# bghira/universal-metal-flash-attention

Hardware: NVIDIA B200
Metric: attention forward TFLOP/s (higher is better)
Workload: dtype bf16

## Files before the change

### universal-metal-flash-attention_b200/csrc/attn_fwd_tc.cu

```cuda
#include <cuda.h>
#include <cuda_runtime.h>
#include <cuda_fp16.h>
#include <math_constants.h>

#include <mutex>
#include <type_traits>

#include "common.h"
#include "fwd_tc.h"
#include "sm100_ptx.cuh"
#include "tc_host.h"

namespace mfa {

namespace {

using namespace ptx;

constexpr int kThreads = 384;
constexpr float kLog2e = 1.4426950408889634f;
constexpr float kLn2 = 0.6931471805599453f;
constexpr float kRescaleThreshold = 8.f;
constexpr int kTileNoMask = 1 << 30;
constexpr int kParts = 4;

template <int D, int MODE, int MASKED = 0>
struct Cfg {
  static constexpr bool kI4 = MODE == kFwdI4 || MODE == kFwdI4F8;
  static constexpr bool kF8 = MODE == kFwdI8F8 || MODE == kFwdI4F8;
  static constexpr bool kI8 = MODE == kFwdI8 || kF8 || kI4;
  static constexpr bool kSplit = MODE == kFwdSplit;
  static constexpr bool kWide = MODE == kFwdWideF16 || MODE == kFwdWideBF16;
  static constexpr int kChunkBytes = 128 * 128;
  static constexpr int kQChunks = kI8 ? 1 : D / 64;
  static constexpr int kVChunks = kF8 ? 1 : D / 64;
  static constexpr int kHalf = kQChunks * kChunkBytes;
  static constexpr int kQTile = kHalf * ((kSplit || kWide) ? 2 : 1);
  static constexpr int kVTile = kVChunks * kChunkBytes;
  static constexpr int kStage = kVTile;
  static constexpr int kSPS = kSplit ? 4 : kWide ? 3 : 2;
  static constexpr bool kMaskTma = MASKED == 2 && (MODE == kFwdF16 || MODE == kFwdBF16);
  static constexpr int kMaskTile = 128 * 128 * 2;
  static constexpr bool kShallow = MASKED != 0 && !kI4;
  static constexpr int kStages = (kSplit || kWide) ? 3
                               : (D == 128 && !kF8) ? (kShallow ? 3 : 5) : (kShallow ? 6 : 10);
  static constexpr int kBarBytes = 112 + 16 * kStages + 16 + 16 + 64 + 32;
  static constexpr int kPoly = kSplit ? 0 : 3;
  static constexpr int kRawTile = 128 * 64, kRawStages = 3;
  static constexpr int kRawBytes = kI4 ? (kRawStages + 1) * kRawTile + 1024 + 128 : 0;
  static constexpr int kMaskBytes = kMaskTma ? 2 * kMaskTile + 1024 : 0;
  static constexpr int kSmem = 2 * kQTile + kStages * kStage + kBarBytes + kRawBytes + kMaskBytes + 1024;
  static_assert(kSmem <= 232448, "shared memory budget of one CTA");
};

__device__ __forceinline__ f32x2 exp2_poly2(f32x2 x) {
  float x0, x1;
  unpack2(x, x0, x1);
  x = pack2(fmaxf(x0, -127.f), fmaxf(x1, -127.f));
  const f32x2 magic = pack2(12582912.f, 12582912.f);
  const f32x2 xr = add2_rm(x, magic);
  const f32x2 f = sub2(x, sub2(xr, magic));
  f32x2 pz = fma2(f, pack2(0.07706582f, 0.07706582f), pack2(0.22764632f, 0.22764632f));
  pz = fma2(pz, f, pack2(0.69511649f, 0.69511649f));
  pz = fma2(pz, f, pack2(1.0f, 1.0f));
  float p0, p1, r0, r1;
  unpack2(pz, p0, p1);
  unpack2(xr, r0, r1);
  return pack2(__int_as_float(__float_as_int(p0) + (__float_as_int(r0) << 23)),
               __int_as_float(__float_as_int(p1) + (__float_as_int(r1) << 23)));
}

template <int PF, int NP>
__device__ __forceinline__ void exp_part(const float* s, f32x2 a2, f32x2 nk2, uint32_t* pk, f32x2& acc_a, f32x2& acc_b) {
  static_assert(NP == 0 || NP == 3, "exp2 mixes: all MUFU, or pairs 1, 4, 6 of every 8 on the polynomial");
  constexpr int kSel = NP == 3 ? 0x52 : 0x00;
  uint32_t half16[PF == 2 ? 16 : 1];
#pragma unroll
  for (int i = 0; i < 16; ++i) {
    const f32x2 x = fma2(pack2(s[2 * i], s[2 * i + 1]), a2, nk2);
    f32x2 pp;
    float p0, p1;
    if ((kSel >> (i & 7)) & 1) {
      pp = exp2_poly2(x);
    } else {
      float x0, x1;
      unpack2(x, x0, x1);
      pp = pack2(ex2(x0), ex2(x1));
    }
    if (i & 1) acc_b = add2(acc_b, pp); else acc_a = add2(acc_a, pp);
    unpack2(pp, p0, p1);
    if constexpr (PF == 2) half16[i] = pack_e4m3(p0, p1);
    else if constexpr (PF == 3) {
      const uint32_t h = pack_f16(p0, p1);
      const float2 hf = __half22float2(*reinterpret_cast<const __half2*>(&h));
      pk[i] = h;
      pk[16 + i] = pack_f16(p0 - hf.x, p1 - hf.y);
    }
    else pk[i] = PF == 1 ? pack_bf16(p0, p1) : pack_f16(p0, p1);
  }
  if constexpr (PF == 2) {
#pragma unroll
    for (int i = 0; i < 8; ++i) pk[i] = half16[2 * i] | (half16[2 * i + 1] << 16);
  }
}

template <int PF, int NP>
__device__ __forceinline__ void exp_phase(const float* s, float a0, float a1, float nk0, float nk1, uint32_t tS,
                                          uint32_t bar0, int lane, float& sum_lo, float& sum_hi) {
  constexpr int kW = PF == 2 ? 8 : 16;
  f32x2 acc[2][2] = {{pack2(0.f, 0.f), pack2(0.f, 0.f)}, {pack2(0.f, 0.f), pack2(0.f, 0.f)}};
  uint32_t pk[kParts][PF == 3 ? 32 : kW];
#pragma unroll
  for (int part = 0; part < kParts; ++part) {
    const bool hi = part >= kParts / 2;
    const float ah = hi ? a1 : a0, nk = hi ? nk1 : nk0;
    exp_part<PF, NP>(s + 32 * part, pack2(ah, ah), pack2(nk, nk), pk[part], acc[hi ? 1 : 0][0], acc[hi ? 1 : 0][1]);
    if (part > 0) {
      tmem_wait_st();
      tc_fence_before();
      __syncwarp();
      if (lane == 0) mbar_arrive(bar0 + 8 * (part - 1));
    }
    if constexpr (PF == 2) tmem_st_x8(tS + kW * part, pk[part]);
    else tmem_st_x16(tS + kW * part, pk[part]);
    if constexpr (PF == 3) tmem_st_x16(tS + 64 + kW * part, pk[part] + 16);
  }
  tmem_wait_st();
  tc_fence_before();
  __syncwarp();
  if (lane == 0) mbar_arrive(bar0 + 8 * (kParts - 1));
  float x0, x1;
  unpack2(add2(acc[0][0], acc[0][1]), x0, x1); sum_lo = x0 + x1;
  unpack2(add2(acc[1][0], acc[1][1]), x0, x1); sum_hi = x0 + x1;
}

template <bool BF>
__device__ __forceinline__ void add_mask_pair(float& s0, float& s1, uint32_t w, f32x2 cn2) {
  float lo, hi;
  if constexpr (BF) {
    lo = __uint_as_float(w << 16);
    hi = __uint_as_float(w & 0xffff0000u);
  } else {
    const float2 f = __half22float2(*reinterpret_cast<const __half2*>(&w));
    lo = f.x; hi = f.y;
  }
  unpack2(fma2(pack2(s0, s1), cn2, pack2(lo, hi)), s0, s1);
}

template <int D, int MODE, int MASKED>
__global__ void __launch_bounds__(kThreads, 1) fwd_tc_kernel(const __grid_constant__ FwdTcParams p) {
  using C = Cfg<D, MODE, MASKED>;
  constexpr bool I8 = C::kI8, F8 = C::kF8, SPLIT = C::kSplit, I4 = C::kI4, WIDE = C::kWide, MT = C::kMaskTma;
  constexpr int PF = SPLIT ? 3 : F8 ? 2 : ((MODE == kFwdF16 || MODE == kFwdWideF16) ? 0 : 1);
  constexpr float kShift = F8 ? 6.f : 0.f;
  constexpr float kThr = F8 ? 2.f : kRescaleThreshold;
  constexpr int QT = C::kQTile, HT = C::kHalf, VT = C::kVTile, STG = C::kStage, NS = C::kStages, CHB = C::kChunkBytes;
  constexpr int SPS = C::kSPS;
  constexpr int kWg2Regs = 40;
  extern __shared__ uint8_t smem_raw[];
  const uint32_t raw = smem_u32(smem_raw);
  const uint32_t base = (raw + 1023u) & ~1023u;
  const uint32_t sQ = base, sKV = base + 2 * QT, sBar = sKV + NS * STG;
  auto q_full = [&](int t) { return sBar + 8 * t; };
  auto s_full = [&](int t) { return sBar + 16 + 8 * t; };
  auto o_full = [&](int t) { return sBar + 32 + 8 * t; };
  auto p_part = [&](int t, int k) { return sBar + 48 + 8 * (t * kParts + k); };
  auto kv_full = [&](int s) { return sBar + 112 + 8 * s; };
  auto kv_empty = [&](int s) { return sBar + 112 + 8 * NS + 8 * s; };
  const uint32_t tmem_slot = sBar + 112 + 16 * NS;
  auto o_empty = [&](int t) { return sBar + 112 + 16 * NS + 16 + 8 * t; };
  constexpr int NR = C::kRawStages, RAW = C::kRawTile;
  auto raw_full = [&](int s) { return sBar + 112 + 16 * NS + 32 + 8 * s; };
  auto raw_empty = [&](int s) { return sBar + 112 + 16 * NS + 56 + 8 * s; };
  const uint32_t qraw_full = sBar + 112 + 16 * NS + 80, qraw_empty = sBar + 112 + 16 * NS + 88;
  const uint32_t sRawK = (sBar + C::kBarBytes + 127u) & ~127u, sRawQ = sRawK + NR * RAW, sQsum = sRawQ + RAW;
  auto mk_full = [&](int t) { return sBar + 112 + 16 * NS + 96 + 8 * t; };
  auto mk_empty = [&](int t) { return sBar + 112 + 16 * NS + 112 + 8 * t; };
  const uint32_t sMask = (sBar + C::kBarBytes + 1023u) & ~1023u;

  const int warp = __shfl_sync(0xffffffffu, threadIdx.x >> 5, 0), lane = threadIdx.x & 31;
  const int* const seg_q = MASKED ? nullptr : p.cu_q;
  const int* const seg_k = MASKED ? nullptr : p.cu_k;
  struct Item { int r0, h, b, hk, nt, j_lo, n, lid, half; };
  auto decode = [&](int w) {
    const int nqb = (p.Sq + 255) / 256;
    Item it;
    it.half = 0;
    if constexpr (WIDE) { it.half = w & 1; w >>= 1; }
    const int x = w % nqb, hb = w / nqb;
    const int qblk = p.causal ? nqb - 1 - x : x;
    it.h = hb % p.H; it.b = hb / p.H;
    it.hk = it.h / (p.H / p.Hkv);
    it.r0 = qblk * 256;
    it.nt = (it.r0 + 128 < p.Sq) ? 2 : 1;
    int klo, khi;
    block_key_range(p.causal, p.window, p.Sq, p.Skv, seg_q, seg_k, p.nseq, it.r0, min(it.r0 + 256, p.Sq), klo, khi);
    it.j_lo = klo >> 7;
    it.n = khi > klo ? ((khi + 127) >> 7) - it.j_lo : 0;
    it.lid = 0;
    if constexpr (MASKED) {
      if (p.mtiles) {
        it.lid = ((p.mask_sb ? it.b : 0) * (p.mask_sh ? p.H : 1) + (p.mask_sh ? it.h : 0)) * nqb + qblk;
        it.n = __ldg(p.mcounts + it.lid);
      }
    }
    return it;
  };
  auto tile_of = [&](const Item& im, int it) {
    if constexpr (MASKED) { if (p.mtiles) return __ldg(p.mtiles + (size_t)im.lid * p.m_nkt + it); }
    return im.j_lo + it;
  };

  if (threadIdx.x == 256) {
    for (int t = 0; t < 2; ++t) {
      mbar_init(q_full(t), 1); mbar_init(s_full(t), 1); mbar_init(o_full(t), 1);
      for (int k = 0; k < kParts; ++k) mbar_init(p_part(t, k), 4);
    }
    for (int s = 0; s < NS; ++s) { mbar_init(kv_full(s), 1); mbar_init(kv_empty(s), 2); }
    for (int t = 0; t < 2; ++t) mbar_init(o_empty(t), 4);
    if constexpr (I4) {
      for (int r = 0; r < NR; ++r) { mbar_init(raw_full(r), 1); mbar_init(raw_empty(r), 1); }
      mbar_init(qraw_full, 1); mbar_init(qraw_empty, 1);
    }
    if constexpr (MT) {
      for (int t = 0; t < 2; ++t) { mbar_init(mk_full(t), 1); mbar_init(mk_empty(t), 4); }
    }
    fence_mbar_init();
  }
  if (warp == 9) {
    if (lane == 0) { prefetch_tmap(&p.tq); prefetch_tmap(&p.tk); prefetch_tmap(&p.tv); }
    __syncwarp();
    tmem_alloc(tmem_slot, 512);
    tmem_relinquish();
  }
  tc_fence_before();
  __syncthreads();
  tc_fence_after();
  const uint32_t tmem = __shfl_sync(0xffffffffu, *reinterpret_cast<volatile uint32_t*>(smem_raw + (tmem_slot - raw)), 0);

  if (warp == 9) {
    reg_dealloc<kWg2Regs>();
    if (lane == 0) {
      const Item im = decode(blockIdx.x);
      const int r0 = im.r0, h = im.h, b = im.b, hk = im.hk, nt = im.nt, n = im.n;
      int kvi = 0;
      int kr = 0, nqraw = 0;
      auto load_half = [&](uint32_t dst, const CUtensorMap* m, uint32_t bar, int row, int head, int col0 = 0) {
#pragma unroll
        for (int c = 0; c < C::kQChunks; ++c) tma_load_4d(dst + c * CHB, m, bar, col0 + c * (I8 ? 128 : 64), row, head, b);
      };
      auto load_q = [&](int t2) {
        if constexpr (I4) {
          if (nqraw > 0) mbar_wait(qraw_empty, (nqraw - 1) & 1);
          mbar_arrive_expect_tx(qraw_full, RAW);
          tma_load_4d(sRawQ, &p.tq, qraw_full, 0, r0 + t2 * 128, h, b);
          ++nqraw;
          return;
        }
        mbar_arrive_expect_tx(q_full(t2), QT);
        load_half(sQ + t2 * QT, &p.tq, q_full(t2), r0 + t2 * 128, h);
        if constexpr (SPLIT) load_half(sQ + t2 * QT + HT, &p.tq2, q_full(t2), r0 + t2 * 128, h);
        if constexpr (WIDE) load_half(sQ + t2 * QT + HT, &p.tq, q_full(t2), r0 + t2 * 128, h, 128);
      };
      auto load_k = [&](const CUtensorMap* m, int row, int col0 = 0) {
        if constexpr (I4) {
          const int rs = kr % NR;
          mbar_wait(raw_empty(rs), ((kr / NR) & 1) ^ 1);
          mbar_arrive_expect_tx(raw_full(rs), RAW);
          tma_load_4d(sRawK + rs * RAW, m, raw_full(rs), 0, row, hk, b);
          ++kr; ++kvi;
          return;
        }
        const int s = kvi % NS;
        mbar_wait(kv_empty(s), ((kvi / NS) & 1) ^ 1);
        mbar_arrive_expect_tx(kv_full(s), HT);
        load_half(sKV + s * STG, m, kv_full(s), row, hk, col0);
        ++kvi;
      };
      auto load_v = [&](const CUtensorMap* m, int row, int col0 = 0) {
        const int s = kvi % NS;
        mbar_wait(kv_empty(s), ((kvi / NS) & 1) ^ 1);
        mbar_arrive_expect_tx(kv_full(s), VT);
#pragma unroll
        for (int c = 0; c < C::kVChunks; ++c) tma_load_4d(sKV + s * STG + c * CHB, m, kv_full(s), col0 + c * 64, row, hk, b);
        ++kvi;
      };
      if (n > 0) load_q(0);
      for (int it = 0; it < n; ++it) {
        const int row = (tile_of(im, it) & (kTileNoMask - 1)) * 128;
        if constexpr (SPLIT) load_k(&p.tk2, row);
        load_k(&p.tk, row);
        if constexpr (WIDE) load_k(&p.tk, row, 128);
        if (it == 0 && nt == 2) load_q(1);
        load_v(&p.tv, row, WIDE ? 128 * im.half : 0);
        if constexpr (SPLIT) load_v(&p.tv2, row);
      }
    }
  } else if (warp == 8 || warp == 10) {
    reg_dealloc<kWg2Regs>();
    const int t = (warp - 8) >> 1;
    constexpr uint32_t FMT = (PF == 0 || PF == 3) ? 0u : 1u;
    constexpr uint32_t IDESC_S = I4 ? make_idesc(2, 1, 0, 0, 0, 128, 128)
                               : I8 ? make_idesc(2, 1, 1, 0, 0, 128, 128)
                                    : make_idesc(1, FMT, FMT, 0, 0, 128, 128);
    constexpr uint32_t IDESC_O = F8 ? make_idesc(1, 0, 0, 0, 1, 128, D)
                                    : make_idesc(1, FMT, FMT, 0, 1, 128, D);
    const uint32_t q_lo = desc_lo(sQ, 16) + t * (QT >> 4), k_lo = desc_lo(sKV, 16), v_lo = desc_lo(sKV, CHB);
    const uint32_t tS = tmem + t * 128, tO = tmem + 256 + t * D;
    auto wait_full = [&](int idx) { mbar_wait(kv_full(idx % NS), (idx / NS) & 1); };
    auto issue_qk = [&](uint32_t a0, int idx, bool acc0) {
      const uint32_t b0 = k_lo + (idx % NS) * (STG >> 4);
#pragma unroll
      for (int kk = 0; kk < D / 16; ++kk) {
        const uint32_t off = ((kk >> 2) * CHB + (kk & 3) * 32) >> 4;
        mma_f16_ss_u(tS, a0 + off, kDescHiSw128, b0 + off, kDescHiSw128, IDESC_S, acc0 || kk > 0);
      }
    };
    auto issue_s = [&](int idx) {
      const uint32_t b0 = k_lo + (idx % NS) * (STG >> 4);
      if constexpr (I8) {
#pragma unroll
        for (int kk = 0; kk < 4; ++kk)
          mma_i8_ss_u(tS, q_lo + kk * 2, kDescHiSw128, b0 + kk * 2, kDescHiSw128, IDESC_S, kk > 0);
      } else {
        issue_qk(q_lo, idx, false);
      }
    };
    auto issue_o_part = [&](int idx, int part, bool acc) {
      const uint32_t b0 = v_lo + (idx % NS) * (STG >> 4);
      if constexpr (F8) {
        mma_f8_ts_u(tO, tS + part * 8, b0 + part * (4096 >> 4), kDescHiSw128, IDESC_O, (acc || part > 0) ? 1u : 0u);
      } else {
#pragma unroll
        for (int kk = 2 * part; kk < 2 * part + 2; ++kk) {
          mma_f16_ts_u(tO, tS + kk * 8, b0 + kk * (2048 >> 4), kDescHiSw128, IDESC_O, (acc || kk > 0) ? 1u : 0u);
          if constexpr (SPLIT) mma_f16_ts_u(tO, tS + 64 + kk * 8, b0 + kk * (2048 >> 4), kDescHiSw128, IDESC_O, 1u);
        }
      }
    };
    int pc = 0;
    int oe = 0;
    const int F = SPLIT ? p.flush_steps : 0;
    const Item im = decode(blockIdx.x);
    const int nt = im.nt, n = im.n;
    if (n > 0 && t < nt) {
      auto release = [&](int idx) { tc_commit_u(kv_empty(idx % NS)); if (nt == 1) tc_commit_u(kv_empty(idx % NS)); };
      auto do_s = [&](int idx) {
        wait_full(idx);
        tc_fence_after();
        if constexpr (SPLIT) {
          issue_qk(q_lo, idx, false);
          release(idx);
          wait_full(idx + 1);
          tc_fence_after();
          issue_qk(q_lo, idx + 1, true);
          issue_qk(q_lo + (HT >> 4), idx + 1, true);
          tc_commit_u(s_full(t));
          release(idx + 1);
        } else if constexpr (WIDE) {
          issue_qk(q_lo, idx, false);
          release(idx);
          wait_full(idx + 1);
          tc_fence_after();
          issue_qk(q_lo + (HT >> 4), idx + 1, true);
          tc_commit_u(s_full(t));
          release(idx + 1);
        } else {
          issue_s(idx);
          tc_commit_u(s_full(t));
          release(idx);
        }
      };
      mbar_wait(q_full(t), 0);
      do_s(0);
      for (int it = 0; it < n; ++it) {
        const int vi = SPS * it + (SPS == 2 ? 1 : 2), ki = SPS * (it + 1);
        wait_full(vi);
#pragma unroll
        for (int part = 0; part < kParts; ++part) {
          mbar_wait(p_part(t, part), pc & 1);
          const bool fresh = F > 0 ? (it % F == 0) : (it == 0);
          if (part == 0 && fresh && it > 0) { mbar_wait(o_empty(t), oe & 1); ++oe; }
          tc_fence_after();
          issue_o_part(vi, part, !fresh);
        }
        release(vi);
        if constexpr (SPLIT) {
          wait_full(vi + 1);
          tc_fence_after();
          const uint32_t b0 = v_lo + ((vi + 1) % NS) * (STG >> 4);
#pragma unroll
          for (int kk = 0; kk < 8; ++kk) mma_f16_ts_u(tO, tS + kk * 8, b0 + kk * (2048 >> 4), kDescHiSw128, IDESC_O, 1u);
          release(vi + 1);
        }
        if (it + 1 < n) do_s(ki);
        else tc_commit_u(o_full(t));
        ++pc;
      }
    }
  } else if (warp < 8) {
    reg_alloc<232>();
    const int t = warp >> 2;
    const int row = (warp & 3) * 32 + lane;
    const uint32_t lane_base = (uint32_t)((warp & 3) * 32) << 16;
    const uint32_t tS = tmem + lane_base + t * 128;
    const uint32_t tO = tmem + lane_base + 256 + t * D;
    int pc = 0;
    int mkc = 0;
    if (t == 1) named_bar_arrive(2, 256);
    const Item im = decode(blockIdx.x);
    const int r0 = im.r0, h = im.h, b = im.b, hk = im.hk, nt = im.nt, n = im.n;
    const int r = r0 + t * 128 + row;
    float m = -CUDART_INF_F, l = 0.f;
    int clo, chi;
    row_key_range(p.causal, p.window, p.Sq, p.Skv, seg_q, seg_k, p.nseq, r, clo, chi);
    --chi;
    float qsc = p.c;
    const float* ksp = nullptr;
    const float* vsp = nullptr;
    if constexpr (I8) {
      const int rq = min(r, p.Sq - 1);
      qsc = (p.qs ? p.qs[((size_t)b * p.H + h) * p.sq_ + rq / p.qbr] : p.qs1) * p.c;
      ksp = p.ks ? p.ks + ((size_t)b * p.Hkv + hk) * p.sk_ : nullptr;
      vsp = p.vs ? p.vs + ((size_t)b * p.Hkv + hk) * p.sv_ : nullptr;
    }
    if constexpr (SPLIT) qsc = p.c * __ldg(p.qs) * __ldg(p.ks);
    float sb_row = p.s_bias;
    float m_flush = -CUDART_INF_F;
    int nflush = 0;
    const int dv_row = p.dv > 0 ? p.dv : D;
    const bool v_blocks = I8 && !F8 && vsp != nullptr;
    const bool pingpong = nt == 2;

    if (t < nt) {
      float ksn0 = p.ks1, ksn1 = p.ks1, vsn0 = 1.f, vsn1 = 1.f;
      int jt_next = n > 0 ? tile_of(im, 0) : 0;
      auto fetch_scales = [&](int jt) {
        if constexpr (I8) {
          const int c0 = (jt & (kTileNoMask - 1)) * 128;
          if (ksp) {
            ksn0 = __ldg(ksp + min(c0 / p.kbr, p.nbk - 1));
            ksn1 = __ldg(ksp + min((c0 + 64) / p.kbr, p.nbk - 1));
// ... 26 lines not shown
        if constexpr (SPLIT) {
          if (p.flush_steps > 0 && it > 0 && it % p.flush_steps == 0) {
            const float fs = (nflush > 0 && m_flush != -CUDART_INF_F) ? ex2(m_flush - m) : 0.f;
            float4* fbuf = reinterpret_cast<float4*>(p.flush_buf) + ((size_t)blockIdx.x * 2 + t) * (size_t)(D / 4) * 128 + row;
#pragma unroll
            for (int ch = 0; ch < D / 32; ++ch) {
              uint32_t ou[32];
              tmem_ld_x32(tO + ch * 32, ou);
              tmem_wait_ld();
#pragma unroll
              for (int i = 0; i < 8; ++i) {
                float4* dst = fbuf + (size_t)(ch * 8 + i) * 128;
                float4 o4 = make_float4(0.f, 0.f, 0.f, 0.f);
                if (nflush > 0) o4 = *dst;
                *dst = make_float4(fmaf(o4.x, fs, __uint_as_float(ou[4 * i])), fmaf(o4.y, fs, __uint_as_float(ou[4 * i + 1])),
                                   fmaf(o4.z, fs, __uint_as_float(ou[4 * i + 2])), fmaf(o4.w, fs, __uint_as_float(ou[4 * i + 3])));
              }
            }
            tc_fence_before();
            __syncwarp();
            if (lane == 0) mbar_arrive(o_empty(t));
            m_flush = m;
            ++nflush;
          }
        }
        if constexpr (I4) {
          if (it == 0) {
            sb_row = p.s_bias + 8.f * (float)(int)ld_shared_u32(sQsum + t * 512 + row * 4);
            cb0 = -sb_row * a0;
            cb1 = -sb_row * a1;
          }
        }
        uint32_t su[128];
        tmem_ld_x32(tS, su);
        tmem_ld_x32(tS + 32, su + 32);
        tmem_ld_x32(tS + 64, su + 64);
        tmem_ld_x32(tS + 96, su + 96);
        tmem_wait_ld();
        float* s = reinterpret_cast<float*>(su);
        if (it + 1 < n) { jt_next = tile_of(im, it + 1); fetch_scales(jt_next); }
        if constexpr (I8) {
          const int smul = p.s_mul;
          const uint32_t sadd = p.s_add;
#pragma unroll
          for (int i = 0; i < 128; ++i) su[i] = su[i] * smul + sadd;
        }
        if (MT && !mask_noop) {
          if constexpr (MT) {
            mbar_wait(mk_full(t), mkc & 1);
            ++mkc;
            const uint32_t mrow = sMask + (uint32_t)t * C::kMaskTile + (uint32_t)row * 128u;
            const uint32_t sw = (uint32_t)(row & 7);
            if (p.mask_kind == kMaskBool) {
#pragma unroll
              for (int j = 0; j < 8; ++j) {
                float f0, f1, f2, f3;
                ld_shared_v4(mrow + (((uint32_t)j ^ sw) << 4), f0, f1, f2, f3);
                const uint32_t w4[4] = {__float_as_uint(f0), __float_as_uint(f1), __float_as_uint(f2), __float_as_uint(f3)};
#pragma unroll
                for (int k = 0; k < 16; ++k)
                  if (((w4[k >> 2] >> (8 * (k & 3))) & 0xffu) == 0) s[16 * j + k] = -CUDART_INF_F;
              }
            } else {
              const float cn = a0 * kLn2;
              const f32x2 cn2 = pack2(cn, cn);
              auto apply = [&](auto is_bf) {
#pragma unroll
                for (int g = 0; g < 2; ++g) {
#pragma unroll
                  for (int j = 0; j < 8; ++j) {
// ... 90 lines not shown
                if (bf) apply(std::true_type{}); else apply(std::false_type{});
                a0 = a1 = kLog2e;
                cb0 = cb1 = 0.f;
                mask_folded = true;
              } else if (ncol == 128 && (reinterpret_cast<uintptr_t>(mp) & 31) == 0) {
#pragma unroll
                for (int g = 0; g < 2; ++g) {
                  uint32_t w[4][8];
#pragma unroll
                  for (int k4 = 0; k4 < 4; ++k4) ldg256(mp + 16 * (4 * g + k4), w[k4]);
                  const float ah = g == 0 ? a0 : a1, cbh = g == 0 ? cb0 : cb1;
#pragma unroll
                  for (int k4 = 0; k4 < 4; ++k4) {
                    const int c = 4 * g + k4;
#pragma unroll
                    for (int k = 0; k < 8; ++k) {
                      s[16 * c + 2 * k] = fmaf(s[16 * c + 2 * k], ah, fmaf(widen(w[k4][k] & 0xffffu), kLog2e, cbh));
                      s[16 * c + 2 * k + 1] = fmaf(s[16 * c + 2 * k + 1], ah, fmaf(widen(w[k4][k] >> 16), kLog2e, cbh));
                    }
                  }
                }
              } else {
#pragma unroll
                for (int i = 0; i < 128; ++i)
                  s[i] = fmaf(s[i], i < 64 ? a0 : a1, fmaf(i < ncol ? widen(__ldg(mp + i)) : 0.f, kLog2e, i < 64 ? cb0 : cb1));
              }
            }
            if (!mask_folded) {
              a0 = a1 = 1.f;
              cb0 = cb1 = 0.f;
            }
          }
        }
        const bool need_mask = (c0 < clo) || (c0 + 127 > chi);
        const bool any_mask = __any_sync(0xffffffffu, need_mask);
        if (any_mask) {
          const int lo_i = clo - c0, hi_i = chi - c0;
#pragma unroll
          for (int i = 0; i < 128; ++i) s[i] = (i < lo_i || i > hi_i) ? -CUDART_INF_F : s[i];
        }
        float mxa = s[0], mxb = s[1], mxc = s[64], mxd = s[65];
#pragma unroll
        for (int i = 2; i < 64; i += 2) {
          mxa = fmaxf(mxa, s[i]); mxb = fmaxf(mxb, s[i + 1]); mxc = fmaxf(mxc, s[64 + i]); mxd = fmaxf(mxd, s[65 + i]);
        }
        float mx;
        if constexpr (I8) mx = fmaxf(fmaf(fmaxf(mxa, mxb), a0, cb0), fmaf(fmaxf(mxc, mxd), a1, cb1));
        else mx = fmaxf(fmaxf(mxa, mxb), fmaxf(mxc, mxd)) * a0;
        float m_new = fmaxf(m, mx);
        const bool grow = (m_new - m) > kThr;
        if (!grow) m_new = m;
        if (__any_sync(0xffffffffu, grow)) {
          const float alpha = grow ? ex2(m - m_new) : 1.f;
          l *= alpha;
          if (it > 0) {
#pragma unroll
            for (int ch = 0; ch < D / 16; ++ch) {
              uint32_t ou[16];
              tmem_ld_x16(tO + ch * 16, ou);
              tmem_wait_ld();
#pragma unroll
              for (int i = 0; i < 16; ++i) ou[i] = __float_as_uint(__uint_as_float(ou[i]) * alpha);
              tmem_st_x16(tO + ch * 16, ou);
            }
          }
        }
        m = m_new;
        const float mm = (m == -CUDART_INF_F) ? 0.f : m;
        const float nk0 = (lv0 - mm) + (cb0 + kShift), nk1 = (lv1 - mm) + (cb1 + kShift);
        float sum_lo, sum_hi;
        if (pingpong) {
          if (t == 0) named_bar_sync(2, 256);
          else named_bar_sync(3, 256);
        }
        exp_phase<PF, C::kPoly>(s, a0, a1, nk0, nk1, tS, p_part(t, 0), lane, sum_lo, sum_hi);
        if (pingpong) {
          if (t == 0) named_bar_arrive(3, 256);
          else named_bar_arrive(2, 256);
        }
        l += sum_lo * iv0 + sum_hi * iv1;
      }
      if (n > 0) {
        mbar_wait(o_full(t), 0);
        tc_fence_after();
      }
      float inv = (l > 0.f ? 1.f / l : 0.f) * ((I8 && !v_blocks) ? p.vs1 : 1.f);
      if constexpr (F8) { if (p.vs) inv = (l > 0.f ? 1.f / l : 0.f) * __ldg(p.vs + (size_t)b * p.Hkv + hk); }
      if constexpr (SPLIT) inv *= __ldg(p.vs);
      const bool live = r < p.Sq;
      const bool padded_d = p.dv > 0 && p.dv < (WIDE ? 256 : D);
      const int dv_tile = p.dv - (WIDE ? 128 * im.half : 0);
      const size_t orow = (size_t)b * p.o_sb + (size_t)h * p.o_sh + (size_t)r * p.o_ss + (WIDE ? 128 * im.half : 0);
      const size_t lrow = ((size_t)b * p.H + h) * p.lse_sh + r;
      float l_out = l > 0.f ? m + log2f(l) - kShift : -CUDART_INF_F;
      float c_old = 0.f;
      const bool acc_mode = p.accumulate && p.o_dtype == kF32;
      const bool tma_out = p.o_tma && !acc_mode;
      if (tma_out) {
        if (n > 0 && nt == 2) { mbar_wait(o_full(t ^ 1), 0); tc_fence_after(); }
      }
      if (acc_mode && live) {
        const float l_old = p.lse[lrow];
        const float mx = fmaxf(l_old, l_out);
        if (mx != -CUDART_INF_F) {
          const float w_old = exp2f(l_old - mx), w_new = exp2f(l_out - mx);
          const float tot = w_old + w_new;
          c_old = w_old / tot;
          inv *= w_new / tot;
          l_out = mx + log2f(tot);
        }
      }
#pragma unroll
      uint32_t oall[D];
      if (n > 0) {
#pragma unroll
        for (int ch = 0; ch < D / 32; ++ch) tmem_ld_x32(tO + ch * 32, oall + ch * 32);
        tmem_wait_ld();
        if constexpr (SPLIT) {
          if (nflush > 0) {
            const float fs = m_flush != -CUDART_INF_F ? ex2(m_flush - m) : 0.f;
            const float4* src = reinterpret_cast<const float4*>(p.flush_buf) + ((size_t)blockIdx.x * 2 + t) * (size_t)(D / 4) * 128 + row;
#pragma unroll
            for (int i = 0; i < D / 4; ++i) {
              const float4 g4 = src[(size_t)i * 128];
              oall[4 * i] = __float_as_uint(fmaf(g4.x, fs, __uint_as_float(oall[4 * i])));
              oall[4 * i + 1] = __float_as_uint(fmaf(g4.y, fs, __uint_as_float(oall[4 * i + 1])));
              oall[4 * i + 2] = __float_as_uint(fmaf(g4.z, fs, __uint_as_float(oall[4 * i + 2])));
              oall[4 * i + 3] = __float_as_uint(fmaf(g4.w, fs, __uint_as_float(oall[4 * i + 3])));
            }
          }
        }
      } else {
#pragma unroll
        for (int i = 0; i < D; ++i) oall[i] = 0u;
      }
#pragma unroll
      for (int ch = 0; ch < D / 32; ++ch) {
        const uint32_t* ou = oall + ch * 32;
        if (tma_out && p.o_dtype == kF32) {
          const uint32_t line = base + (uint32_t)(t * (D / 32) + ch) * (128u * 128u) + (uint32_t)row * 128u;
#pragma unroll
          for (int i = 0; i < 8; ++i)
            st_shared_v4(line + (uint32_t)((i ^ (row & 7)) << 4), __uint_as_float(ou[4 * i]) * inv, __uint_as_float(ou[4 * i + 1]) * inv,
                         __uint_as_float(ou[4 * i + 2]) * inv, __uint_as_float(ou[4 * i + 3]) * inv);
        } else if (tma_out) {
          const uint32_t line = base + (uint32_t)(t * (D / 64) + (ch >> 1)) * (128u * 128u) + (uint32_t)row * 128u;
#pragma unroll
          for (int i = 0; i < 4; ++i) {
            uint32_t w[4];
#pragma unroll
            for (int k = 0; k < 4; ++k) {
              const float a = __uint_as_float(ou[8 * i + 2 * k]) * inv, bb = __uint_as_float(ou[8 * i + 2 * k + 1]) * inv;
              w[k] = p.o_dtype == kBF16 ? pack_bf16(a, bb) : pack_f16(a, bb);
            }
            const int unit = (ch & 1) * 4 + i;
            st_shared_v4(line + (uint32_t)((unit ^ (row & 7)) << 4), __uint_as_float(w[0]), __uint_as_float(w[1]),
                         __uint_as_float(w[2]), __uint_as_float(w[3]));
          }
        } else if (live && padded_d) {
          const int nv = dv_tile - ch * 32;
#pragma unroll
          for (int i = 0; i < 32; ++i) {
            if (i >= nv) continue;
            const float val = __uint_as_float(ou[i]) * inv;
            if (p.o_dtype == kF32) {
              float* dst = reinterpret_cast<float*>(p.o) + orow + ch * 32 + i;
              *dst = acc_mode ? fmaf(*dst, c_old, val) : val;
            } else {
              uint16_t* dst = reinterpret_cast<uint16_t*>(p.o) + orow + ch * 32 + i;
              *dst = (uint16_t)((p.o_dtype == kBF16 ? pack_bf16(val, 0.f) : pack_f16(val, 0.f)) & 0xffffu);
            }
// ... 13 lines not shown
            } else if (acc_mode) {
              float4 old[8];
#pragma unroll
              for (int i = 0; i < 8; ++i) old[i] = dst[i];
#pragma unroll
              for (int i = 0; i < 8; ++i)
                dst[i] = make_float4(fmaf(old[i].x, c_old, __uint_as_float(ou[4 * i]) * inv),
                                     fmaf(old[i].y, c_old, __uint_as_float(ou[4 * i + 1]) * inv),
                                     fmaf(old[i].z, c_old, __uint_as_float(ou[4 * i + 2]) * inv),
                                     fmaf(old[i].w, c_old, __uint_as_float(ou[4 * i + 3]) * inv));
            } else {
#pragma unroll
              for (int i = 0; i < 8; ++i)
                dst[i] = make_float4(__uint_as_float(ou[4 * i]) * inv, __uint_as_float(ou[4 * i + 1]) * inv,
                                     __uint_as_float(ou[4 * i + 2]) * inv, __uint_as_float(ou[4 * i + 3]) * inv);
            }
          } else {
            uint4* dst = reinterpret_cast<uint4*>(reinterpret_cast<uint16_t*>(p.o) + orow + ch * 32);
#pragma unroll
            for (int i = 0; i < 4; ++i) {
              uint32_t w[4];
#pragma unroll
              for (int k = 0; k < 4; ++k) {
                const float a = __uint_as_float(ou[8 * i + 2 * k]) * inv, bb = __uint_as_float(ou[8 * i + 2 * k + 1]) * inv;
                w[k] = p.o_dtype == kBF16 ? pack_bf16(a, bb) : pack_f16(a, bb);
              }
              dst[i] = make_uint4(w[0], w[1], w[2], w[3]);
            }
          }
        }
      }
      if (tma_out) {
        fence_proxy_async_smem();
        named_bar_sync(4 + t, 128);
        if ((threadIdx.x & 127) == 0) {
          if (p.o_dtype == kF32) {
#pragma unroll
            for (int ch = 0; ch < D / 32; ++ch)
              tma_store_4d(&p.to, base + (uint32_t)(t * (D / 32) + ch) * (128u * 128u), ch * 32 + (WIDE ? 128 * im.half : 0), r0 + t * 128, h, b);
          } else {
#pragma unroll
            for (int ch = 0; ch < D / 64; ++ch)
              tma_store_4d(&p.to, base + (uint32_t)(t * (D / 64) + ch) * (128u * 128u), ch * 64 + (WIDE ? 128 * im.half : 0), r0 + t * 128, h, b);
          }
          bulk_commit();
          bulk_wait_read();
        }
      }
      if (live && p.lse && (!WIDE || im.half == 0)) p.lse[lrow] = l_out;
    }
    if (t == 0) named_bar_sync(2, 256);
  }
  else {
    reg_dealloc<kWg2Regs>();
    if constexpr (MT) {
      if (lane == 0) {
        prefetch_tmap(&p.tm);
        const uint64_t pol = l2_policy_evict_first();
        const bool one_byte = p.mask_kind == kMaskBool;
        int mc[2] = {0, 0};
        const Item im = decode(blockIdx.x);
        const int mb = p.mask_sb ? im.b : 0, mh = p.mask_sh ? im.h : 0;
        for (int it = 0; it < im.n; ++it) {
          const int jt = tile_of(im, it);
          if (jt & kTileNoMask) continue;
          const int c0 = (jt & (kTileNoMask - 1)) * 128;
          for (int t = 0; t < im.nt; ++t) {
            if (mc[t] > 0) mbar_wait(mk_empty(t), (mc[t] - 1) & 1);
            const uint32_t dst = sMask + (uint32_t)t * C::kMaskTile;
            if (one_byte) {
              mbar_arrive_expect_tx(mk_full(t), 16384);
              tma_load_4d_hint(dst, &p.tm, mk_full(t), c0, im.r0 + t * 128, mh, mb, pol);
            } else {
              mbar_arrive_expect_tx(mk_full(t), 32768);
              tma_load_4d_hint(dst, &p.tm, mk_full(t), c0, im.r0 + t * 128, mh, mb, pol);
              tma_load_4d_hint(dst + 16384, &p.tm, mk_full(t), c0 + 64, im.r0 + t * 128, mh, mb, pol);
            }
            ++mc[t];
          }
        }
      }
    }
    if constexpr (I4) {
      auto unpack_tile = [&](uint32_t src, uint32_t dst, auto is_q, uint32_t qsum_addr) {
// ... 26 lines not shown
            rs += __shfl_xor_sync(0xffffffffu, rs, 1);
            rs += __shfl_xor_sync(0xffffffffu, rs, 2);
            if (su == 0) st_shared_u32(qsum_addr + row * 4, (uint32_t)rs);
          }
        }
      };
      int kr = 0, cq = 0;
      const Item im = decode(blockIdx.x);
      const int nt = im.nt, n = im.n;
      auto convert_q = [&](int t2) {
        mbar_wait(qraw_full, cq & 1);
        unpack_tile(sRawQ, sQ + t2 * QT, std::true_type{}, sQsum + t2 * 512);
        fence_proxy_async_smem();
        __syncwarp();
        if (lane == 0) { mbar_arrive(q_full(t2)); mbar_arrive(qraw_empty); }
        ++cq;
      };
      if (n > 0) convert_q(0);
      for (int it = 0; it < n; ++it) {
        const int idx = 2 * it, s = idx % NS, rs = kr % NR;
        mbar_wait(raw_full(rs), (kr / NR) & 1);
        mbar_wait(kv_empty(s), ((idx / NS) & 1) ^ 1);
        unpack_tile(sRawK + rs * RAW, sKV + s * STG, std::false_type{}, 0u);
        fence_proxy_async_smem();
        __syncwarp();
        if (lane == 0) { mbar_arrive(kv_full(s)); mbar_arrive(raw_empty(rs)); }
        ++kr;
        if (it == 0 && nt == 2) convert_q(1);
      }
    }
  }
  tc_fence_before();
  __syncthreads();
  if (warp == 9) tmem_dealloc(*reinterpret_cast<volatile uint32_t*>(smem_raw + (tmem_slot - raw)), 512);
}

struct MaskTileParams {
  const void* mask;
  int kind, scalar;
  long long sb, sh, sq;
  int Sq, Skv, causal, window, nqb, nkt, MH;
  int* tiles;
  int* counts;
};

template <bool WARP_TILE>
__global__ void __launch_bounds__(WARP_TILE ? 256 : 64, WARP_TILE ? 4 : 16) mask_flags_kernel(const MaskTileParams q, uint8_t* __restrict__ flags) {
  const int warp = threadIdx.x >> 5, lane = threadIdx.x & 31;
  const int j = WARP_TILE ? blockIdx.x * 8 + warp : blockIdx.x, qb = blockIdx.y, mbh = blockIdx.z;
  if (j >= q.nkt) return;
  const int mb = mbh / q.MH, mh = mbh % q.MH;
  const int r0 = qb * 256, rows = min(256, q.Sq - r0);
  constexpr int NW = WARP_TILE ? 1 : 2, RPW = 4;
  const int wt = WARP_TILE ? 0 : warp;
  int klo, khi;
  visible_key_range(q.causal, q.window, q.Skv, r0, min(r0 + 256, q.Sq), klo, khi);
  const int j_lo = klo >> 7, j_hi = khi > klo ? (khi + 127) >> 7 : j_lo;
  int any = 0, all = 1;
  if (j >= j_lo && j < j_hi) {
    const int c0 = j * 128, ncol = min(128, q.Skv - c0);
    const int nrows = q.sq ? rows : 1;
    const int esz_sel = q.kind == kMaskBool ? 0 : q.scalar == kMaskF32 ? 2 : 1;
    auto round = [&](int rb, auto nr_tag) {
      constexpr int NR = decltype(nr_tag)::value;
      uint32_t raw[NR][4];
#pragma unroll
      for (int i = 0; i < NR; ++i) {
// ... 94 lines not shown
void launch_flags(const MaskTileParams& q, const M& m, uint8_t* flags, cudaStream_t st) {
  const long long tiles = (long long)m.nkt * m.nqb * m.MB * m.MH;
  if (tiles >= 4096)
    mask_flags_kernel<true><<<dim3((unsigned)((m.nkt + 7) / 8), (unsigned)m.nqb, (unsigned)(m.MB * m.MH)), 256, 0, st>>>(q, flags);
  else
    mask_flags_kernel<false><<<dim3((unsigned)m.nkt, (unsigned)m.nqb, (unsigned)(m.MB * m.MH)), 64, 0, st>>>(q, flags);
}

__global__ void mask_compact_kernel(const uint8_t* __restrict__ flags, int* __restrict__ tiles, int* __restrict__ counts,
                                    int lists, int nkt) {
  const int lid = blockIdx.x * blockDim.x + threadIdx.x;
  if (lid >= lists) return;
  int cnt = 0;
  for (int j = 0; j < nkt; ++j)
    if (const int f = flags[(size_t)lid * nkt + j]) tiles[(size_t)lid * nkt + cnt++] = j | (f == 2 ? kTileNoMask : 0);
  counts[lid] = cnt;
}

using tc::encode_fn;
using tc::make_map;

bool view_ok(const TensorView& t, int64_t, int64_t Hn, int64_t B) { return tc::view_ok(t, Hn, B); }

template <int D, int MODE, int MASKED>
cudaError_t launch_k(const FwdTcParams& prm, dim3 grid, cudaStream_t st) {
  static bool attr_set = false;
  auto kern = fwd_tc_kernel<D, MODE, MASKED>;
  constexpr int kSmem = Cfg<D, MODE, MASKED>::kSmem;
  if (!attr_set) {
    cudaError_t e = cudaFuncSetAttribute(kern, cudaFuncAttributeMaxDynamicSharedMemorySize, kSmem);
    if (e != cudaSuccess) return e;
    attr_set = true;
  }
  kern<<<grid, kThreads, kSmem, st>>>(prm);
  return cudaGetLastError();
}

template <int D, int MODE>
cudaError_t launch(const FwdTcParams& prm, dim3 grid, cudaStream_t st) {
  if (!prm.mask) return launch_k<D, MODE, 0>(prm, grid, st);
  if constexpr (Cfg<D, MODE, 2>::kMaskTma) {
    if (prm.mask_tma) return launch_k<D, MODE, 2>(prm, grid, st);
  }
  return launch_k<D, MODE, 1>(prm, grid, st);
}

}

cudaError_t launch_fwd_tc_kernel(const FwdTcParams& prm_in, int D, int mode, cudaStream_t st, int B) {
  FwdTcParams prm = prm_in;
  prm.nbatch = B;
  ptx::watchdog_bind();
  const bool wide = mode == kFwdWideF16 || mode == kFwdWideBF16;
  const long long items = (long long)((prm.Sq + 255) / 256) * prm.H * B * (wide ? 2 : 1);
  if (items <= 0 || items > 0x7fffffffLL) return cudaErrorInvalidValue;
  const dim3 grid((unsigned)items, 1, 1);
  if (wide) {
    if (D != 256) return cudaErrorInvalidValue;
    return mode == kFwdWideBF16 ? launch<128, kFwdWideBF16>(prm, grid, st) : launch<128, kFwdWideF16>(prm, grid, st);
  }
  if (D == 64 && mode == kFwdBF16) return launch<64, kFwdBF16>(prm, grid, st);
  if (D == 64 && mode == kFwdF16) return launch<64, kFwdF16>(prm, grid, st);
  if (D != 128) return cudaErrorInvalidValue;
  switch (mode) {
    case kFwdF16: return launch<128, kFwdF16>(prm, grid, st);
    case kFwdBF16: return launch<128, kFwdBF16>(prm, grid, st);
    case kFwdI8: return launch<128, kFwdI8>(prm, grid, st);
// ... 141 lines not shown
```

Baseline: 1194.

## Split softmax key columns across two warpgroups per tile in unmasked f16/bf16

For unmasked f16/bf16 forward, the number of softmax warps doubles from 8 to 16. Each row's 128 key scores and D output columns are split between two warpgroups, which exchange partial row max and row sum through a small shared-memory slot guarded by named barriers. The aim is to cut the per-thread exp/max work and register pressure on the softmax critical path. In exchange it adds per-iteration barrier synchronisation and fewer registers per softmax thread, and it drops one K/V pipeline stage to fit the extra shared memory.

```diff
diff --git a/universal-metal-flash-attention_b200/csrc/attn_fwd_tc.cu b/universal-metal-flash-attention_b200/csrc/attn_fwd_tc.cu
--- a/universal-metal-flash-attention_b200/csrc/attn_fwd_tc.cu
+++ b/universal-metal-flash-attention_b200/csrc/attn_fwd_tc.cu
@@ -17,7 +17,6 @@
 
 using namespace ptx;
 
-constexpr int kThreads = 384;
 constexpr float kLog2e = 1.4426950408889634f;
 constexpr float kLn2 = 0.6931471805599453f;
 constexpr float kRescaleThreshold = 8.f;
@@ -42,14 +41,22 @@
   static constexpr bool kMaskTma = MASKED == 2 && (MODE == kFwdF16 || MODE == kFwdBF16);
   static constexpr int kMaskTile = 128 * 128 * 2;
   static constexpr bool kShallow = MASKED != 0 && !kI4;
+  static constexpr bool kKeySplit = (MODE == kFwdF16 || MODE == kFwdBF16) && MASKED == 0;
+  static constexpr int kSoftWarps = kKeySplit ? 16 : 8;
+  static constexpr int kThreads = 32 * kSoftWarps + 128;
+  static constexpr int kSoftRegs = kKeySplit ? 112 : 232;
+  static constexpr int kOtherRegs = kKeySplit ? 32 : 40;
+  static_assert((kThreads / 128 - 1) * kSoftRegs + kOtherRegs <= (kThreads / 128) * (65536 / kThreads / 8 * 8),
+                "setmaxnreg.inc would wait for registers no warpgroup gives back");
   static constexpr int kStages = (kSplit || kWide) ? 3
-                               : (D == 128 && !kF8) ? (kShallow ? 3 : 5) : (kShallow ? 6 : 10);
+                               : (D == 128 && !kF8) ? (kShallow ? 3 : kKeySplit ? 4 : 5) : (kShallow ? 6 : 10);
   static constexpr int kBarBytes = 112 + 16 * kStages + 16 + 16 + 64 + 32;
+  static constexpr int kXBytes = kKeySplit ? 2 * 2 * 128 * 2 * 4 : 0;
   static constexpr int kPoly = kSplit ? 0 : 3;
   static constexpr int kRawTile = 128 * 64, kRawStages = 3;
   static constexpr int kRawBytes = kI4 ? (kRawStages + 1) * kRawTile + 1024 + 128 : 0;
   static constexpr int kMaskBytes = kMaskTma ? 2 * kMaskTile + 1024 : 0;
-  static constexpr int kSmem = 2 * kQTile + kStages * kStage + kBarBytes + kRawBytes + kMaskBytes + 1024;
+  static constexpr int kSmem = 2 * kQTile + kStages * kStage + kBarBytes + kXBytes + kRawBytes + kMaskBytes + 1024;
   static_assert(kSmem <= 232448, "shared memory budget of one CTA");
 };
 
@@ -104,15 +111,15 @@
   }
 }
 
-template <int PF, int NP>
+template <int PF, int NP, int NPT = kParts>
 __device__ __forceinline__ void exp_phase(const float* s, float a0, float a1, float nk0, float nk1, uint32_t tS,
                                           uint32_t bar0, int lane, float& sum_lo, float& sum_hi) {
   constexpr int kW = PF == 2 ? 8 : 16;
   f32x2 acc[2][2] = {{pack2(0.f, 0.f), pack2(0.f, 0.f)}, {pack2(0.f, 0.f), pack2(0.f, 0.f)}};
-  uint32_t pk[kParts][PF == 3 ? 32 : kW];
-#pragma unroll
-  for (int part = 0; part < kParts; ++part) {
-    const bool hi = part >= kParts / 2;
+  uint32_t pk[NPT][PF == 3 ? 32 : kW];
+#pragma unroll
+  for (int part = 0; part < NPT; ++part) {
+    const bool hi = part >= NPT / 2;
     const float ah = hi ? a1 : a0, nk = hi ? nk1 : nk0;
     exp_part<PF, NP>(s + 32 * part, pack2(ah, ah), pack2(nk, nk), pk[part], acc[hi ? 1 : 0][0], acc[hi ? 1 : 0][1]);
     if (part > 0) {
@@ -128,7 +135,7 @@
   tmem_wait_st();
   tc_fence_before();
   __syncwarp();
-  if (lane == 0) mbar_arrive(bar0 + 8 * (kParts - 1));
+  if (lane == 0) mbar_arrive(bar0 + 8 * (NPT - 1));
   float x0, x1;
   unpack2(add2(acc[0][0], acc[0][1]), x0, x1); sum_lo = x0 + x1;
   unpack2(add2(acc[1][0], acc[1][1]), x0, x1); sum_hi = x0 + x1;
@@ -148,19 +155,23 @@
 }
 
 template <int D, int MODE, int MASKED>
-__global__ void __launch_bounds__(kThreads, 1) fwd_tc_kernel(const __grid_constant__ FwdTcParams p) {
+__global__ void __launch_bounds__(Cfg<D, MODE, MASKED>::kThreads, 1) fwd_tc_kernel(const __grid_constant__ FwdTcParams p) {
   using C = Cfg<D, MODE, MASKED>;
   constexpr bool I8 = C::kI8, F8 = C::kF8, SPLIT = C::kSplit, I4 = C::kI4, WIDE = C::kWide, MT = C::kMaskTma;
+  constexpr bool KS = C::kKeySplit;
+  constexpr int SW = C::kSoftWarps;
+  constexpr int GT = 16 * SW;
   constexpr int PF = SPLIT ? 3 : F8 ? 2 : ((MODE == kFwdF16 || MODE == kFwdWideF16) ? 0 : 1);
   constexpr float kShift = F8 ? 6.f : 0.f;
   constexpr float kThr = F8 ? 2.f : kRescaleThreshold;
   constexpr int QT = C::kQTile, HT = C::kHalf, VT = C::kVTile, STG = C::kStage, NS = C::kStages, CHB = C::kChunkBytes;
   constexpr int SPS = C::kSPS;
-  constexpr int kWg2Regs = 40;
+  constexpr int kWg2Regs = C::kOtherRegs;
   extern __shared__ uint8_t smem_raw[];
   const uint32_t raw = smem_u32(smem_raw);
   const uint32_t base = (raw + 1023u) & ~1023u;
-  const uint32_t sQ = base, sKV = base + 2 * QT, sBar = sKV + NS * STG;
+  const uint32_t sQ = base, sKV = base + 2 * QT;
+  uint32_t sBar = sKV + NS * STG;
   auto q_full = [&](int t) { return sBar + 8 * t; };
   auto s_full = [&](int t) { return sBar + 16 + 8 * t; };
   auto o_full = [&](int t) { return sBar + 32 + 8 * t; };
@@ -177,6 +188,8 @@
   auto mk_full = [&](int t) { return sBar + 112 + 16 * NS + 96 + 8 * t; };
   auto mk_empty = [&](int t) { return sBar + 112 + 16 * NS + 112 + 8 * t; };
   const uint32_t sMask = (sBar + C::kBarBytes + 1023u) & ~1023u;
+  auto x_slot = [&](int t, int row, int half) { return sBar + C::kBarBytes + (uint32_t)((t * 128 + row) * 8 + 4 * half); };
+  constexpr uint32_t kXPar = 2 * 128 * 8;
 
   const int warp = __shfl_sync(0xffffffffu, threadIdx.x >> 5, 0), lane = threadIdx.x & 31;
   const int* const seg_q = MASKED ? nullptr : p.cu_q;
@@ -211,7 +224,7 @@
     return im.j_lo + it;
   };
 
-  if (threadIdx.x == 256) {
+  if (threadIdx.x == 32 * SW) {
     for (int t = 0; t < 2; ++t) {
       mbar_init(q_full(t), 1); mbar_init(s_full(t), 1); mbar_init(o_full(t), 1);
       for (int k = 0; k < kParts; ++k) mbar_init(p_part(t, k), 4);
@@ -227,7 +240,7 @@
     }
     fence_mbar_init();
   }
-  if (warp == 9) {
+  if (warp == SW + 1) {
     if (lane == 0) { prefetch_tmap(&p.tq); prefetch_tmap(&p.tk); prefetch_tmap(&p.tv); }
     __syncwarp();
     tmem_alloc(tmem_slot, 512);
@@ -237,8 +250,9 @@
   __syncthreads();
   tc_fence_after();
   const uint32_t tmem = __shfl_sync(0xffffffffu, *reinterpret_cast<volatile uint32_t*>(smem_raw + (tmem_slot - raw)), 0);
-
-  if (warp == 9) {
+  uint32_t tmem_free = ~0u;
+
+  if (warp == SW + 1) {
     reg_dealloc<kWg2Regs>();
     if (lane == 0) {
       const Item im = decode(blockIdx.x);
@@ -296,9 +310,13 @@
         if constexpr (SPLIT) load_v(&p.tv2, row);
       }
     }
-  } else if (warp == 8 || warp == 10) {
+    tmem_free = tmem;
+  } else if (warp == SW || warp == SW + 2) {
     reg_dealloc<kWg2Regs>();
-    const int t = (warp - 8) >> 1;
+    if constexpr (KS) asm volatile("add.u32 %0, %1, %2;" : "=r"(sBar) : "r"(base), "n"(2 * QT + NS * STG));
+    const Item im = decode(blockIdx.x);
+    const int nt = im.nt, n = im.n;
+    const int t = (warp - SW) >> 1;
     constexpr uint32_t FMT = (PF == 0 || PF == 3) ? 0u : 1u;
     constexpr uint32_t IDESC_S = I4 ? make_idesc(2, 1, 0, 0, 0, 128, 128)
                                : I8 ? make_idesc(2, 1, 1, 0, 0, 128, 128)
@@ -341,8 +359,6 @@
     int pc = 0;
     int oe = 0;
     const int F = SPLIT ? p.flush_steps : 0;
-    const Item im = decode(blockIdx.x);
-    const int nt = im.nt, n = im.n;
     if (n > 0 && t < nt) {
       auto release = [&](int idx) { tc_commit_u(kv_empty(idx % NS)); if (nt == 1) tc_commit_u(kv_empty(idx % NS)); };
       auto do_s = [&](int idx) {
@@ -398,16 +414,21 @@
         ++pc;
       }
     }
-  } else if (warp < 8) {
-    reg_alloc<232>();
-    const int t = warp >> 2;
+  } else if (warp < SW) {
+    reg_alloc<C::kSoftRegs>();
+    const int t = warp / (SW / 2);
+    const int kh = KS ? (warp >> 2) & 1 : 0;
     const int row = (warp & 3) * 32 + lane;
     const uint32_t lane_base = (uint32_t)((warp & 3) * 32) << 16;
     const uint32_t tS = tmem + lane_base + t * 128;
     const uint32_t tO = tmem + lane_base + 256 + t * D;
+    constexpr int NSC = KS ? 64 : 128;
+    constexpr int OC = KS ? D / 2 : D;
+    const int k_off = 64 * kh, o_off = OC * kh;
+    const uint32_t xs_own = x_slot(t, row, kh);
     int pc = 0;
     int mkc = 0;
-    if (t == 1) named_bar_arrive(2, 256);
+    if (t == 1) named_bar_arrive(2, 2 * GT);
     const Item im = decode(blockIdx.x);
     const int r0 = im.r0, h = im.h, b = im.b, hk = im.hk, nt = im.nt, n = im.n;
     const int r = r0 + t * 128 + row;
@@ -500,10 +521,8 @@
           }
         }
         uint32_t su[128];
-        tmem_ld_x32(tS, su);
-        tmem_ld_x32(tS + 32, su + 32);
-        tmem_ld_x32(tS + 64, su + 64);
-        tmem_ld_x32(tS + 96, su + 96);
+#pragma unroll
+        for (int c = 0; c < NSC / 32; ++c) tmem_ld_x32(tS + k_off + 32 * c, su + 32 * c);
         tmem_wait_ld();
         float* s = reinterpret_cast<float*>(su);
         if (it + 1 < n) { jt_next = tile_of(im, it + 1); fetch_scales(jt_next); }
@@ -660,21 +679,36 @@
             }
           }
         }
-        const bool need_mask = (c0 < clo) || (c0 + 127 > chi);
+        const int k0 = c0 + k_off;
+        const bool need_mask = (k0 < clo) || (k0 + NSC - 1 > chi);
         const bool any_mask = __any_sync(0xffffffffu, need_mask);
         if (any_mask) {
-          const int lo_i = clo - c0, hi_i = chi - c0;
-#pragma unroll
-          for (int i = 0; i < 128; ++i) s[i] = (i < lo_i || i > hi_i) ? -CUDART_INF_F : s[i];
-        }
-        float mxa = s[0], mxb = s[1], mxc = s[64], mxd = s[65];
-#pragma unroll
-        for (int i = 2; i < 64; i += 2) {
-          mxa = fmaxf(mxa, s[i]); mxb = fmaxf(mxb, s[i + 1]); mxc = fmaxf(mxc, s[64 + i]); mxd = fmaxf(mxd, s[65 + i]);
+          const int lo_i = clo - k0, hi_i = chi - k0;
+#pragma unroll
+          for (int i = 0; i < NSC; ++i) s[i] = (i < lo_i || i > hi_i) ? -CUDART_INF_F : s[i];
         }
         float mx;
-        if constexpr (I8) mx = fmaxf(fmaf(fmaxf(mxa, mxb), a0, cb0), fmaf(fmaxf(mxc, mxd), a1, cb1));
-        else mx = fmaxf(fmaxf(mxa, mxb), fmaxf(mxc, mxd)) * a0;
+        if constexpr (KS) {
+          float mxa = s[0], mxb = s[1];
+#pragma unroll
+          for (int i = 2; i < 64; i += 2) { mxa = fmaxf(mxa, s[i]); mxb = fmaxf(mxb, s[i + 1]); }
+          const uint32_t xs = xs_own + (it & 1) * kXPar;
+          st_shared_u32(xs, __float_as_uint(fmaxf(mxa, mxb) * a0));
+          tc_fence_before();
+          named_bar_sync(6 + t, GT);
+          tc_fence_after();
+          float mx0, mx1;
+          ld_shared_v2(xs & ~7u, mx0, mx1);
+          mx = fmaxf(mx0, mx1);
+        } else {
+          float mxa = s[0], mxb = s[1], mxc = s[64], mxd = s[65];
+#pragma unroll
+          for (int i = 2; i < 64; i += 2) {
+            mxa = fmaxf(mxa, s[i]); mxb = fmaxf(mxb, s[i + 1]); mxc = fmaxf(mxc, s[64 + i]); mxd = fmaxf(mxd, s[65 + i]);
+          }
+          if constexpr (I8) mx = fmaxf(fmaf(fmaxf(mxa, mxb), a0, cb0), fmaf(fmaxf(mxc, mxd), a1, cb1));
+          else mx = fmaxf(fmaxf(mxa, mxb), fmaxf(mxc, mxd)) * a0;
+        }
         float m_new = fmaxf(m, mx);
         const bool grow = (m_new - m) > kThr;
         if (!grow) m_new = m;
@@ -683,13 +717,19 @@
           l *= alpha;
           if (it > 0) {
 #pragma unroll
-            for (int ch = 0; ch < D / 16; ++ch) {
+            for (int ch = 0; ch < OC / 16; ++ch) {
               uint32_t ou[16];
-              tmem_ld_x16(tO + ch * 16, ou);
+              tmem_ld_x16(tO + o_off + ch * 16, ou);
               tmem_wait_ld();
 #pragma unroll
               for (int i = 0; i < 16; ++i) ou[i] = __float_as_uint(__uint_as_float(ou[i]) * alpha);
-              tmem_st_x16(tO + ch * 16, ou);
+              tmem_st_x16(tO + o_off + ch * 16, ou);
+            }
+            if constexpr (KS) {
+              tmem_wait_st();
+              tc_fence_before();
+              named_bar_sync(8 + 4 * t + (row >> 5), 64);
+              tc_fence_after();
             }
           }
         }
@@ -698,13 +738,16 @@
         const float nk0 = (lv0 - mm) + (cb0 + kShift), nk1 = (lv1 - mm) + (cb1 + kShift);
         float sum_lo, sum_hi;
         if (pingpong) {
-          if (t == 0) named_bar_sync(2, 256);
-          else named_bar_sync(3, 256);
-        }
-        exp_phase<PF, C::kPoly>(s, a0, a1, nk0, nk1, tS, p_part(t, 0), lane, sum_lo, sum_hi);
+          if (t == 0) named_bar_sync(2, 2 * GT);
+          else named_bar_sync(3, 2 * GT);
+        }
+        if constexpr (KS)
+          exp_phase<PF, C::kPoly, 2>(s, a0, a0, nk0, nk0, tS + 32 * kh, p_part(t, 2 * kh), lane, sum_lo, sum_hi);
+        else
+          exp_phase<PF, C::kPoly>(s, a0, a1, nk0, nk1, tS, p_part(t, 0), lane, sum_lo, sum_hi);
         if (pingpong) {
-          if (t == 0) named_bar_arrive(3, 256);
-          else named_bar_arrive(2, 256);
+          if (t == 0) named_bar_arrive(3, 2 * GT);
+          else named_bar_arrive(2, 2 * GT);
         }
         l += sum_lo * iv0 + sum_hi * iv1;
       }
@@ -712,23 +755,33 @@
         mbar_wait(o_full(t), 0);
         tc_fence_after();
       }
+      const bool live = r < p.Sq;
+      const size_t lrow = ((size_t)b * p.H + h) * p.lse_sh + r;
+      const bool acc_mode = p.accumulate && p.o_dtype == kF32;
+      float l_old = 0.f;
+      if constexpr (KS) {
+        if (acc_mode && live) l_old = p.lse[lrow];
+        const uint32_t xs = xs_own + (n & 1) * kXPar;
+        st_shared_u32(xs, __float_as_uint(l));
+        named_bar_sync(6 + t, GT);
+        float l0, l1;
+        ld_shared_v2(xs & ~7u, l0, l1);
+        l = l0 + l1;
+      }
       float inv = (l > 0.f ? 1.f / l : 0.f) * ((I8 && !v_blocks) ? p.vs1 : 1.f);
       if constexpr (F8) { if (p.vs) inv = (l > 0.f ? 1.f / l : 0.f) * __ldg(p.vs + (size_t)b * p.Hkv + hk); }
       if constexpr (SPLIT) inv *= __ldg(p.vs);
-      const bool live = r < p.Sq;
       const bool padded_d = p.dv > 0 && p.dv < (WIDE ? 256 : D);
       const int dv_tile = p.dv - (WIDE ? 128 * im.half : 0);
       const size_t orow = (size_t)b * p.o_sb + (size_t)h * p.o_sh + (size_t)r * p.o_ss + (WIDE ? 128 * im.half : 0);
-      const size_t lrow = ((size_t)b * p.H + h) * p.lse_sh + r;
       float l_out = l > 0.f ? m + log2f(l) - kShift : -CUDART_INF_F;
       float c_old = 0.f;
-      const bool acc_mode = p.accumulate && p.o_dtype == kF32;
       const bool tma_out = p.o_tma && !acc_mode;
       if (tma_out) {
         if (n > 0 && nt == 2) { mbar_wait(o_full(t ^ 1), 0); tc_fence_after(); }
       }
       if (acc_mode && live) {
-        const float l_old = p.lse[lrow];
+        if constexpr (!KS) l_old = p.lse[lrow];
         const float mx = fmaxf(l_old, l_out);
         if (mx != -CUDART_INF_F) {
           const float w_old = exp2f(l_old - mx), w_new = exp2f(l_out - mx);
@@ -738,11 +791,10 @@
           l_out = mx + log2f(tot);
         }
       }
-#pragma unroll
-      uint32_t oall[D];
+      uint32_t oall[OC];
       if (n > 0) {
 #pragma unroll
-        for (int ch = 0; ch < D / 32; ++ch) tmem_ld_x32(tO + ch * 32, oall + ch * 32);
+        for (int ch = 0; ch < OC / 32; ++ch) tmem_ld_x32(tO + o_off + ch * 32, oall + ch * 32);
         tmem_wait_ld();
         if constexpr (SPLIT) {
           if (nflush > 0) {
@@ -760,11 +812,12 @@
         }
       } else {
 #pragma unroll
-        for (int i = 0; i < D; ++i) oall[i] = 0u;
-      }
-#pragma unroll
-      for (int ch = 0; ch < D / 32; ++ch) {
-        const uint32_t* ou = oall + ch * 32;
+        for (int i = 0; i < OC; ++i) oall[i] = 0u;
+      }
+#pragma unroll
+      for (int cl = 0; cl < OC / 32; ++cl) {
+        const int ch = o_off / 32 + cl;
+        const uint32_t* ou = oall + cl * 32;
         if (tma_out && p.o_dtype == kF32) {
           const uint32_t line = base + (uint32_t)(t * (D / 32) + ch) * (128u * 128u) + (uint32_t)row * 128u;
 #pragma unroll
@@ -844,8 +897,8 @@
       }
       if (tma_out) {
         fence_proxy_async_smem();
-        named_bar_sync(4 + t, 128);
-        if ((threadIdx.x & 127) == 0) {
+        named_bar_sync(4 + t, GT);
+        if (threadIdx.x % GT == 0) {
           if (p.o_dtype == kF32) {
 #pragma unroll
             for (int ch = 0; ch < D / 32; ++ch)
@@ -859,9 +912,9 @@
           bulk_wait_read();
         }
       }
-      if (live && p.lse && (!WIDE || im.half == 0)) p.lse[lrow] = l_out;
+      if (live && p.lse && (!WIDE || im.half == 0) && kh == 0) p.lse[lrow] = l_out;
     }
-    if (t == 0) named_bar_sync(2, 256);
+    if (t == 0) named_bar_sync(2, 2 * GT);
   }
   else {
     reg_dealloc<kWg2Regs>();
@@ -954,7 +1007,7 @@
   }
   tc_fence_before();
   __syncthreads();
-  if (warp == 9) tmem_dealloc(*reinterpret_cast<volatile uint32_t*>(smem_raw + (tmem_slot - raw)), 512);
+  if (tmem_free != ~0u) tmem_dealloc(tmem_free, 512);
 }
 
 struct MaskTileParams {
@@ -1115,7 +1168,7 @@
     if (e != cudaSuccess) return e;
     attr_set = true;
   }
-  kern<<<grid, kThreads, kSmem, st>>>(prm);
+  kern<<<grid, Cfg<D, MODE, MASKED>::kThreads, kSmem, st>>>(prm);
   return cudaGetLastError();
 }
 
```

Result: slower. 1138 (median of 6 runs) (-4.7%).
